# evroon/mav-detection

Measured on AMD Instinct MI355X. Metric: frame-pairs/sec at 1920x1080, higher is better.
Workload: dtype f32; 1 GPU; 1920x1080, batch 64 per GPU, Farneback + FoE + phi/threshold + box; global_batch=64, parallelism=frame-parallel x1, record_exchange=none (1 GPU), torch_in_process=False

## Files before the change

### include/mavflow.h

```cpp
#ifndef MAVFLOW_H
#define MAVFLOW_H

#include <stddef.h>
#include <stdint.h>

#ifdef __cplusplus
extern "C" {
#endif

#define MAV_OK 0
#define MAV_ERR_ARG (-1)
#define MAV_ERR_HIP (-2)
#define MAV_ERR_OOM (-3)
#define MAV_ERR_STATE (-4)

#define MAV_DEPTH_8U 0
#define MAV_DEPTH_16U 2
#define MAV_DEPTH_32F 5

typedef struct mav_ctx mav_ctx;

#define MAV_OPTFLOW_USE_INITIAL_FLOW 4
#define MAV_OPTFLOW_FARNEBACK_GAUSSIAN 256
typedef struct {
// ... 219 lines not shown
                            float* corners, int* count);
int mav_good_features_score_dev(mav_ctx*, const uint8_t* gray_dev, const uint8_t* mask_dev, const mav_gftt_params*, const mav_corner_score*,
                                float* corners_dev, int32_t* count_dev);
int mav_gftt_last_pick(mav_ctx*, uint32_t* stats);
#define MAV_LK_HIST_BINS 104
int mav_lk_last_iterations(mav_ctx*, uint32_t* hist);
int mav_lk_level_dims(const mav_ctx*, int level, int* w, int* h);

int mav_timer_start(mav_ctx*);
int mav_timer_stop(mav_ctx*, float* ms);
int mav_profile_enable(mav_ctx*, int on);
int mav_profile_get(mav_ctx*, int* n, const char** names, double* total_ms, long* launches);
int mav_profile_busy(mav_ctx*, const char* names, double* busy_ms);
int mav_profile_intervals(mav_ctx*, int* n, int* kernel_class, int* stream, float* t0_ms, float* t1_ms);

int mav_membw_probe(mav_ctx*, size_t bytes_per_buffer, int reps, double* gbs);

int mav_runtime_info(char* buf, size_t cap);
int mav_comm_unique_id(void* id128 );
int mav_comm_init(mav_ctx*, const void* id128, int rank, int nranks, void** comm_out);
int mav_comm_count(void* comm, int* nranks);
int mav_comm_destroy(void* comm);
int mav_allgather_results(mav_ctx*, void* comm, const void* local_dev, size_t bytes_per_rank, void* all_dev);

int mav_stage_blur_resize(mav_ctx*, const uint8_t* img, int k, float* out);
int mav_stage_blur_resize_two_pass(mav_ctx*, const uint8_t* img, int k, float* out);
int mav_stage_blur_resize_ex(mav_ctx*, const void* img, int depth, int k, int two_pass, float* out);
int mav_stage_polyexp(mav_ctx*, const float* I, int k, float* R);
int mav_stage_update_matrices(mav_ctx*, const float* R0, const float* R1, const float* flow, int k, float* M);
int mav_stage_update_matrices_from(mav_ctx*, const float* R0, const float* R1, const float* flow_coarse, int k, float* M);
int mav_stage_initial_flow(mav_ctx*, const float* flow0, int k, float* out);
int mav_stage_blur_iter(mav_ctx*, const float* R0, const float* R1, const float* M, int k, int update, float* flow,
                        float* M_out);

int mav_stage_phi_mask(mav_ctx*, const float* flow, const double* foe, const double* omega, const double* dt, const uint8_t* sky,
                       int batch, const mav_thr_params*, double* phi, uint8_t* mask_fixed, uint8_t* mask_dyn, int32_t* box);

int mav_stage_coefficients(mav_ctx*, int k, float* g, float* xg, float* xxg, float* ig, float* blur_taps);

int mav_stage_pyramid_level(mav_ctx*, const uint8_t* img, double scale, int level, uint8_t* out);

int mav_stage_lk_pyramid(mav_ctx*, const uint8_t* img, int level, uint8_t* out);
int mav_stage_lk_scharr(mav_ctx*, const uint8_t* img, int level, int16_t* out);
int mav_stage_min_eigen(mav_ctx*, const uint8_t* img, int block_size, float* out);
int mav_stage_corner_response(mav_ctx*, const uint8_t* img, int block_size, const mav_corner_score*, float* out);
int mav_stage_corner_pick(mav_ctx*, const uint64_t* keys, int n, const mav_gftt_params*, float* corners, int* count);

#ifdef __cplusplus
}
#endif
#endif
```

### mav-detection_amd/csrc/kernels_flow.hip

```cpp
#include "mavflow_internal.h"

#include <algorithm>
#include <type_traits>

static __device__ __forceinline__ int clampi(int v, int lo, int hi) { return v < lo ? lo : (v > hi ? hi : v); }

struct TileMap { int tiles_x, tiles_y, per_img, n_tiles, strip_w, xcd, ty0; };
static __device__ __forceinline__ bool tile_of_block(const TileMap& tm, int* s, int* tx, int* ty)
{
    const int per = ((int)gridDim.x + 7) >> 3;
    const int tile = tm.xcd ? (int)(blockIdx.x & 7) * per + (int)(blockIdx.x >> 3) : (int)blockIdx.x;
    if (tile >= tm.n_tiles) return false;
    const int img = tile / tm.per_img;
    int tr = tile - img * tm.per_img;
    const int strip_tiles = tm.strip_w * tm.tiles_y;
    const int st = tr / strip_tiles;
    tr -= st * strip_tiles;
    const int x_base = st * tm.strip_w;
    const int sw = min(tm.strip_w, tm.tiles_x - x_base);
    const int row = tr / sw;
    *s = img; *ty = row + tm.ty0; *tx = x_base + tr - row * sw;
    return true;
}
static TileMap make_tile_map(int w, int h, int G, int tile_w, int tile_h, int ty0 = 0, int ty1 = -1, int strip = 0)
// ... 1438 lines not shown
{
    const bool wt = a.write_through && a.do_update;
    const auto k = wt ? k_blur_iter_fast<Win, 6, AL, true> : k_blur_iter_fast<Win, 6, AL, false>;
    hipLaunchKernelGGL(k, dim3(tile_grid(tm)), dim3(256), 0, st, a.M_in, a.M_out, a.M_stride, a.R0, a.R1, a.R_stride, a.w, a.h, tm, win,
                       a.do_update, a.store_flow, a.flow, a.f_stride);
}

template <typename Win>
static void launch_sweep(hipStream_t st, const SweepArgs& a, const Win& win)
{
    const int m = a.winsize / 2;
    if (m == 6 && blur_iter_vec_ok(a)) {
        const TileMap tm = make_tile_map(a.w, a.h, a.G, FT_X, FT_Y, a.ty0, a.ty1, a.strip);
        if (tm.n_tiles == 0) return;
        return launch_sweep_fast<Win, true>(st, tm, a, win);
    }
    if (m == 6 && a.f_stride % 2 == 0 && ((uintptr_t)a.flow & 7) == 0)
        return launch_sweep_fast<Win, false>(st, make_tile_map(a.w, a.h, a.G, FT_X, FT_Y, 0, -1, a.strip), a, win);
    int ext, pitch, plane;
    iter_geometry(m, &ext, &pitch, &plane);
    const size_t lds = sizeof(float) * 5 * (size_t)plane;
    const dim3 grid((a.w + MAV_TILE - 1) / MAV_TILE, (a.h + MAV_TILE - 1) / MAV_TILE, a.G);
    const auto k = m == 6 ? k_blur_iter_generic<Win, 6> : k_blur_iter_generic<Win, 0>;
    hipLaunchKernelGGL(k, grid, dim3(256), lds, st, a.M_in, a.M_out, a.M_stride, a.R0, a.R1, a.R_stride, a.w, a.h, m, pitch, plane, win,
                       a.do_update, a.flow, a.f_stride);
}

void launch_blur_iter(hipStream_t st, const SweepArgs& a)
{
    if (a.gauss) launch_sweep(st, a, GaussWindow{*a.gauss});
    else launch_sweep(st, a, BoxWindow{(float)(1.0 / ((double)a.winsize * a.winsize))});
}

const char* blur_iter_prepare(int winsize)
{
    const size_t lds = blur_iter_lds_bytes(winsize);
    if (lds <= (size_t)64 * 1024) return nullptr;
    hipError_t e = hipFuncSetAttribute((const void*)k_blur_iter_generic<BoxWindow, 0>, hipFuncAttributeMaxDynamicSharedMemorySize, (int)lds);
    if (e == hipSuccess) e = hipFuncSetAttribute((const void*)k_blur_iter_generic<GaussWindow, 0>, hipFuncAttributeMaxDynamicSharedMemorySize, (int)lds);
    return e == hipSuccess ? nullptr : hipGetErrorString(e);
}

__global__ __launch_bounds__(256) void k_probe_r3w1(const float4* __restrict__ a, const float4* __restrict__ b, const float4* __restrict__ c,
                                                    float4* __restrict__ d, size_t n)
{
    for (size_t i = (size_t)blockIdx.x * 256 + threadIdx.x; i < n; i += (size_t)gridDim.x * 256) {
        const float4 x = a[i], y = b[i], z = c[i];
        d[i] = make_float4(x.x + y.x + z.x, x.y + y.y + z.y, x.z + y.z + z.z, x.w + y.w + z.w);
    }
}
void launch_probe_r3w1(hipStream_t st, const float* a, const float* b, const float* c, float* d, size_t n_float4)
{
    hipLaunchKernelGGL(k_probe_r3w1, dim3(256 * 8), dim3(256), 0, st, (const float4*)a, (const float4*)b, (const float4*)c, (float4*)d, n_float4);
}
```

### mav-detection_amd/csrc/mavflow.cpp

```cpp
#include <assert.h>
#include <dlfcn.h>
#include <math.h>
#include <float.h>
#include <stdarg.h>
#include <stdio.h>
#include <stdlib.h>
#include <string.h>

#include <algorithm>
#include <atomic>
#include <condition_variable>
#include <deque>
#include <map>
#include <mutex>
#include <string>
#include <thread>
#include <vector>

#include "mavflow_internal.h"

static thread_local std::string g_err;
static int fail(int code, const char* fmt, ...)
{
    char buf[512];
// ... 305 lines not shown
    mav_fb_params fb;
    hipStream_t stream = nullptr;
    hipStream_t copy_stream = nullptr;
    hipEvent_t copy_done = nullptr, compute_mark = nullptr;
    hipEvent_t gather_done = nullptr;
    struct Stager* stager = nullptr;
    struct Worker* worker = nullptr;
    int upload_threads = 4;
    bool inline_uploads = false;
    int stream_priority = 0;
    const float* last_flow = nullptr;
    const uint8_t *last_mf = nullptr, *last_md = nullptr;
    int last_mask_batch = 0;
    std::vector<Layer> layers;
    PolyCoef pc;
    size_t n0 = 0, n1 = 0;
    struct WorkSet {
        float *Htmp = nullptr;
        float *I = nullptr, *R = nullptr, *Ma = nullptr, *Mb = nullptr, *fc[2] = {nullptr, nullptr};
        float *Ic = nullptr, *Rc = nullptr;
    } ws;
    std::vector<size_t> c_off, c_stride;
    size_t c_total = 0;
    struct DeepSet { float *I = nullptr, *R = nullptr, *Ma = nullptr, *Mb = nullptr, *f[2] = {nullptr, nullptr}; } deep;
    int kd = 0, deep_cap = 0;
    int deep_frac = 6;
    bool deep_batch = true;
    int band_skew = -1;
    int band_phase = 0;
    bool coarse_bands = false;
    int small_g = 0;
    bool small_batch = true;
    int sweep_wt = -1;
    int small_batch_mb = 200;
    int window = MAV_WINDOW_BOX;
    GaussTaps gauss;
    int bands = 1;
    int pairs_in_flight = 2, pif_band_mb = 96;
    bool bands_set = false;
    int bands_auto = 1;
    bool group_fine_set = false;
    hipStream_t pair_stream = nullptr;
    hipEvent_t pif_fork = nullptr, pif_join = nullptr;
    bool share_frames = true;
    int coarse_cache_mb = 220;
    bool share_m = true;
    int coarse_half = 0;
    int strip = 0;
    bool phi_screen = true;
    int phi_yloop = 0;
    size_t htmp_stride = 0;
    DevMem mem;
    bool ws_ready = false;
    float* flow_ws = nullptr;
    float* init_snap = nullptr;
    int init_cap = 0;
    size_t init_stride = 0;
    FoeScratch foe_sc{nullptr, nullptr, nullptr};
    int foe_sc_n = 0;
    double* foe_dev = nullptr;
    int32_t* box_acc = nullptr;
    unsigned long long* u64_scratch = nullptr;
    int* i32_scratch = nullptr;
    DerotParams* derot_dev = nullptr;
    unsigned long long* render_max = nullptr;
    DerotParams* render_derot = nullptr;
// ... 320 lines not shown
}
struct Option {
    const char* name;
    long lo, hi;
    int mav_ctx::*i;
    bool mav_ctx::*b;
    bool in_schedule;
    int (*set)(mav_ctx*, long);
};
static const long kAny = 1L << 40;
static const Option kOptions[] = {
    {"group", 1, 1 << 20, &mav_ctx::group, nullptr, true, set_group},
    {"group_fine", 0, 1 << 20, &mav_ctx::group_fine, nullptr, true, set_group_fine},
    {"bands", 0, 8, &mav_ctx::bands, nullptr, true, set_bands},
    {"pairs_in_flight", 1, 2, &mav_ctx::pairs_in_flight, nullptr, true, nullptr},
    {"band_mb", 8, 1 << 20, &mav_ctx::pif_band_mb, nullptr, true, nullptr},
    {"coarse_cache_mb", 0, 1 << 20, &mav_ctx::coarse_cache_mb, nullptr, true, nullptr},
    {"coarse_half", 0, 1 << 20, &mav_ctx::coarse_half, nullptr, true, nullptr},
    {"share_m", 0, 1, nullptr, &mav_ctx::share_m, true, nullptr},
    {"share_frames", 0, 1, nullptr, &mav_ctx::share_frames, true, nullptr},
    {"strip", 0, 1 << 20, &mav_ctx::strip, nullptr, true, nullptr},
    {"phi_screen", 0, 1, nullptr, &mav_ctx::phi_screen, true, nullptr},
    {"phi_yloop", 0, 1 << 20, &mav_ctx::phi_yloop, nullptr, true, nullptr},
    {"small_batch", 0, 1, nullptr, &mav_ctx::small_batch, true, nullptr},
    {"sweep_write_through", -1, 1, &mav_ctx::sweep_wt, nullptr, true, nullptr},
    {"deep_batch", 0, 1, nullptr, &mav_ctx::deep_batch, true, nullptr},
    {"coarse_bands", 0, 1, nullptr, &mav_ctx::coarse_bands, true, nullptr},
    {"band_phase", 0, 64, &mav_ctx::band_phase, nullptr, true, nullptr},
    {"band_skew", -1, 64, &mav_ctx::band_skew, nullptr, true, nullptr},
    {"deep_frac", 1, 1 << 20, &mav_ctx::deep_frac, nullptr, true, set_deep_frac},
    {"upload_threads", 1, 64, &mav_ctx::upload_threads, nullptr, false, set_upload_threads},
    {"inline_uploads", -kAny, kAny, nullptr, &mav_ctx::inline_uploads, false, set_inline_uploads},
    {"stream_priority", -kAny, kAny, &mav_ctx::stream_priority, nullptr, false, set_stream_priority},
};
static const Option* find_option(const char* name)
{
    for (const Option& o : kOptions) if (!strcmp(o.name, name)) return &o;
    return nullptr;
}
static long option_value(const mav_ctx* c, const Option& o) { return o.i ? (long)(c->*o.i) : (long)(c->*o.b); }
extern "C" int mav_get_option(mav_ctx* c, const char* name, long* value)
{
    if (!c || !name || !value) return fail(MAV_ERR_ARG, "mav_get_option: NULL argument");
    const Option* o = find_option(name);
    if (!o) return fail(MAV_ERR_ARG, "unknown option '%s'", name);
    *value = option_value(c, *o);
    return MAV_OK;
}
extern "C" int mav_set_option(mav_ctx* c, const char* name, long value)
{
    if (!c || !name) return fail(MAV_ERR_ARG, "mav_set_option: NULL argument");
    const Option* o = find_option(name);
    if (!o) return fail(MAV_ERR_ARG, "unknown option '%s'", name);
    if (value < o->lo || value > o->hi) return fail(MAV_ERR_ARG, "option '%s' must be in [%ld, %ld], got %ld", name, o->lo, o->hi, value);
    if (o->set) return o->set(c, value);
    if (o->i) c->*o->i = (int)value; else c->*o->b = value != 0;
    return MAV_OK;
}

static const GaussTaps* window_taps(const mav_ctx* c) { return c->window == MAV_WINDOW_GAUSSIAN ? &c->gauss : nullptr; }
extern "C" int mav_set_window(mav_ctx* c, int window)
{
    if (!c) return fail(MAV_ERR_ARG, "mav_set_window: NULL context");
    if (window != MAV_WINDOW_BOX && window != MAV_WINDOW_GAUSSIAN)
        return fail(MAV_ERR_ARG, "mav_set_window: window must be MAV_WINDOW_BOX (0) or MAV_WINDOW_GAUSSIAN (1), got %d", window);
    HIPCHK(hipSetDevice(c->device));
// ... 431 lines not shown
    const Layer& l = c->layers[k];
    const int T = blur_iter_tile_rows(l.h), I = c->fb.iterations;
    auto wt = [&](int streams) { return c->sweep_wt < 0 ? streams == 2 : c->sweep_wt != 0; };
    int sub = g;
    if (k == 0 && c->group_fine > 0 && c->group_fine < g) sub = c->group_fine;
    if (k > 0 && c->coarse_cache_mb > 0) {
        const size_t ws = (size_t)l.w * l.h * 80, cap = (size_t)c->coarse_cache_mb << 20;
        const int fit = (int)(cap / (ws ? ws : 1));
        if (fit < sub) sub = fit > 1 ? fit : 1;
    }
    bool m_per_sub = sub < g;
    const size_t ws_pair = (size_t)l.w * l.h * 80, band_bytes = (size_t)c->pif_band_mb << 20;
    const bool big_coarse = k > 0 && c->coarse_bands && bands_ok && ws_pair > band_bytes && T / (I + 2) >= 2;
    if (big_coarse) { sub = 1; m_per_sub = true; }
    if (k > 0 && !big_coarse && c->pairs_in_flight == 2 && g >= 2) {
        int half = sub / 2 > 0 ? sub / 2 : 1;
        if (c->coarse_half > 0) half = c->coarse_half;
        if (2 * half > g) half = (g + 1) / 2;
        return {"two sub-groups in flight", half, 2, 1, false, M_SUB, SLOT_ALTERNATE, wt(2)};
    }
    if ((k == 0 || big_coarse) && c->pairs_in_flight == 2 && m_per_sub && sub == 1 && g >= 2) {
        int J = (c->bands_set && k == 0) ? c->bands : (int)((ws_pair + band_bytes - 1) / band_bytes);
        const int Jmax = T / (I + 2);
        if (J > Jmax) J = Jmax;
        if (J < 1) J = 1;
        if (J == 1 || bands_ok)
            return {"two pairs in flight, band-major", 1, 2, J, J > 1 && c->band_phase && J >= c->band_phase, J > 1 ? M_BAND : M_SUB,
                    SLOT_ALTERNATE, wt(2)};
    }
    const int J = (k == 0 && (m_per_sub || g == 1) && sub == 1 && T >= (I + 2) * c->bands && bands_ok) ? c->bands : 1;
    return {"one stream", sub, 1, J, false, m_per_sub ? M_SUB : M_GROUP, (m_per_sub && c->share_m) ? SLOT_FIRST : SLOT_OWN, wt(1)};
}

struct BandRun { float *Ma, *Mb; int kid , J, phase; };
static void sweeps_band_major(mav_ctx* c, hipStream_t st, SweepArgs a, const BandRun& run, const FlowSource* upd)
{
    const int I = c->fb.iterations, T = blur_iter_tile_rows(a.h), phase = run.phase;
    int J = run.J;
    const int NBands = phase ? J + 1 : J;
    auto bound = [&](int j) -> int {
        if (j <= 0) return 0;
        if (j >= NBands) return T;
        if (phase) return (int)((long long)T * (2 * j - 1) / (2 * J));
        int b = (int)((long long)T * j / J) + (c->band_skew < 0 ? (I - 1) / 2 : c->band_skew);
        const int lo = j, hi = T - (NBands - j);
        return b < lo ? lo : (b > hi ? hi : b);
    };
    J = NBands;
    for (int j = 0; j < J; j++) {
        const int a0 = bound(j), a1 = bound(j + 1);
        if (a1 <= a0) continue;
        if (upd) {
            ProfScope ps(c, K_UPDATE, st);
            launch_initial_m(st, {a, run.Ma, a.M_stride, a0 == 0 ? 0 : a0 * 16 - 8, j == J - 1 ? a.h : a1 * 16 + 8}, *upd);
        }
        for (int it = 0; it < I; it++) {
            const int update = it < I - 1;
            int ty0 = a0 - it, ty1 = j == J - 1 ? T : a1 - it;
            if (ty0 < 0) ty0 = 0;
            if (ty1 <= ty0) continue;
            ProfScope ps(c, run.kid, st);
            a.M_in = (it & 1) ? run.Mb : run.Ma; a.M_out = (it & 1) ? run.Ma : run.Mb;
            a.do_update = update; a.store_flow = !update; a.ty0 = ty0; a.ty1 = ty1;
            launch_blur_iter(st, a);
        }
    }
}

struct LayerIO { int k, g; const float *r0, *r1; size_t rs; float* flow; size_t fstride, ms; };
struct MBuffers { float *a, *b; };
static int layer_sweeps(mav_ctx* c, hipStream_t st, const LayerIO& io, const FlowSource& src, const MBuffers& m)
{
    const int k = io.k, g = io.g;
    const Layer& l = c->layers[k];
    const size_t ms = io.ms, rs = io.rs;
    const PairOperands group{io.r0, io.r1, rs, g, l.w, l.h};
    SweepArgs sa{group, m.a, m.b, ms, c->fb.winsize, io.flow, io.fstride, 1, 0};
    sa.strip = c->strip; sa.gauss = window_taps(c);
    const SweepPlan p = plan_sweeps(c, k, g, blur_iter_bands_ok(sa));
    sa.write_through = p.write_through;
    if (p.streams == 2) {
        CHK(ensure_pair_stream(c));
        HIPCHK(hipEventRecord(c->pif_fork, st));
        HIPCHK(hipStreamWaitEvent(c->pair_stream, c->pif_fork, 0));
    }
    if (p.m_build == M_GROUP) {
        ProfScope ps(c, K_UPDATE, st);
        launch_initial_m(st, {group, m.a, ms}, src);
    }
    for (int s0 = 0, i = 0; s0 < g; s0 += p.per_launch, i++) {
        const int gs = g - s0 < p.per_launch ? g - s0 : p.per_launch;
        const bool second = p.streams == 2 && (i & 1);
        const hipStream_t ss = second ? c->pair_stream : st;
        const size_t m_off = p.m_slot == SLOT_OWN ? (size_t)s0 * ms : p.m_slot == SLOT_FIRST ? 0 : (size_t)(i & 1) * p.per_launch * ms;
        sa.R0 = io.r0 + (size_t)s0 * rs; sa.R1 = io.r1 + (size_t)s0 * rs; sa.G = gs;
        sa.flow = io.flow + (size_t)s0 * io.fstride;
        const FlowSource bu = src.from_pair(s0);
        if (p.m_build == M_SUB) {
            ProfScope ps(c, K_UPDATE, ss);
            launch_initial_m(ss, {sa, m.a + m_off, ms}, bu);
        }
        sweeps_band_major(c, ss, sa, {m.a + m_off, m.b + m_off, k == 0 ? K_ITER : K_ITER_COARSE, p.J, p.shift_second && second},
                          p.m_build == M_BAND ? &bu : nullptr);
    }
    if (p.streams == 2) {
        prof_close_stream(c, c->pair_stream); prof_close_stream(c, st);
        HIPCHK(hipEventRecord(c->pif_join, c->pair_stream));
        HIPCHK(hipStreamWaitEvent(st, c->pif_join, 0));
    }
    return MAV_OK;
}

template <typename T>
static void layer_expansions(mav_ctx* c, hipStream_t st, int k, const T* prev, const T* next, int g, bool seq, float* I, float* R,
                             const float** r0, const float** r1)
{
    mav_ctx::WorkSet& w = c->ws;
    const size_t n0 = c->n0;
    const Layer& l = c->layers[k];
    const LayerTarget target{I, n0, blur_of(c, l), l.w, l.h};
    const BlurScratch scratch{w.Htmp, c->htmp_stride};
    auto frames = [&](const T* a, const T* b, int split, int G) { return FrameRun<T>{a, b, split, n0, G, c->W, c->H}; };
    if (seq) {
        { ProfScope ps(c, K_BLUR_RESIZE, st);
          launch_blur_resize(st, frames(prev, nullptr, 0, g + 1), target, scratch); }
        { ProfScope ps(c, K_POLYEXP, st);
          launch_polyexp(st, I, n0, g + 1, l.w, l.h, c->pc, R, 5 * n0); }
        *r0 = R; *r1 = R + 5 * n0;
        return;
    }
    float* R1 = R + 5 * n0 * (size_t)g;
    *r0 = R; *r1 = R1;
    const bool no_tmp = !blur_resize_needs_tmp(frames(prev, next, g, 2 * g), target);
    const bool merge_frames = (no_tmp || 2 * g <= g + 1) && (size_t)2 * g * l.w * l.h * sizeof(float) <= ((size_t)48 << 20);
    if (merge_frames) {
// ... 1530 lines not shown
    const Layer* l;
    CHK(h.fresh_layer(k, &l));
    if (!flow0 || !out) return fail(MAV_ERR_ARG, "mav_stage_initial_flow: NULL argument");
    const size_t n = (size_t)l->w * l->h;
    double scale = 1;
    for (int i = 0; i < k; i++) scale *= c->fb.pyr_scale;
    const float* di = h.in(flow0, 2 * c->n0 * sizeof(float));
    float* dout = h.out(out, 2 * n * sizeof(float));
    CHK(h.staged());
    launch_area_resize_flow(c->stream, di, 2 * c->n0, c->W, c->H, dout, 2 * n, l->w, l->h, 1, scale);
    CHK(check_launch("area_resize_flow"));
    return h.finish();
}
extern "C" int mav_stage_blur_iter(mav_ctx* c, const float* R0, const float* R1, const float* M, int k, int update, float* flow, float* M_out)
{
    HostCall h(c, "mav_stage_blur_iter");
    const Layer* l;
    CHK(h.fresh_layer(k, &l));
    if (!R0 || !R1 || !M || !flow || (update && !M_out)) return fail(MAV_ERR_ARG, "mav_stage_blur_iter: NULL argument");
    const size_t n = (size_t)l->w * l->h;
    const float* d0 = h.in(R0, 5 * n * sizeof(float));
    const float* d1 = h.in(R1, 5 * n * sizeof(float));
    const float* dm = h.in(M, 5 * n * sizeof(float));
    float* dmo = h.scratch<float>(5 * n * sizeof(float));
    float* df = h.out(flow, 2 * n * sizeof(float));
    h.fetch(update ? M_out : nullptr, dmo, 5 * n * sizeof(float));
    CHK(h.staged());
    SweepArgs a{{d0, d1, 5 * n, 1, l->w, l->h}, dm, dmo, 5 * n, c->fb.winsize, df, 2 * n, update, 1};
    a.strip = c->strip; a.gauss = window_taps(c);
    launch_blur_iter(c->stream, a);
    CHK(check_launch("blur_iter"));
    return h.finish();
}

typedef int (*nccl_get_uid_t)(void*);
struct uid128 { char b[128]; };
typedef int (*nccl_init_rank2_t)(void**, int, uid128, int);
typedef int (*nccl_destroy_t)(void*);
typedef int (*nccl_allgather_t)(const void*, void*, size_t, int, void*, hipStream_t);
typedef const char* (*nccl_errstr_t)(int);
static void* g_rccl = nullptr;
static int rccl_sym(const char* name, void** fn)
{
    if (!g_rccl) {
        g_rccl = dlopen("librccl.so.1", RTLD_NOW | RTLD_GLOBAL);
        if (!g_rccl) g_rccl = dlopen("librccl.so", RTLD_NOW | RTLD_GLOBAL);
        if (!g_rccl) return fail(MAV_ERR_STATE, "cannot load RCCL: %s", dlerror());
    }
    *fn = dlsym(g_rccl, name);
    if (!*fn) return fail(MAV_ERR_STATE, "RCCL symbol %s missing", name);
    return MAV_OK;
}
typedef int (*nccl_get_version_t)(int*);
extern "C" int mav_runtime_info(char* buf, size_t cap)
{
    if (!buf || cap < 16) return fail(MAV_ERR_ARG, "mav_runtime_info: NULL argument");
    int rt = 0, drv = 0, nccl = 0;
    if (hipRuntimeGetVersion(&rt) != hipSuccess) rt = -1;
    if (hipDriverGetVersion(&drv) != hipSuccess) drv = -1;
    void* fn = nullptr;
    if (g_rccl && (fn = dlsym(g_rccl, "ncclGetVersion"))) ((nccl_get_version_t)fn)(&nccl);
    snprintf(buf, cap, "{\"built_with_hip\": \"%d.%d.%d\", \"hip_runtime\": %d, \"hip_runtime_major\": %d, \"hip_driver\": %d, \"rccl\": %d}",
             HIP_VERSION_MAJOR, HIP_VERSION_MINOR, HIP_VERSION_PATCH, rt, rt > 0 ? rt / 10000000 : -1, drv, nccl);
    return MAV_OK;
}
extern "C" int mav_comm_unique_id(void* id128)
// ... 479 lines not shown
```

### mav-detection_amd/csrc/mavflow_internal.h

```cpp
#pragma once
#include <hip/hip_runtime.h>
#include <stdint.h>

#include "../../include/mavflow.h"

#define MAV_MAX_POLY_N 16
#define MAV_TILE 32

struct PolyCoef {
    int n;
    float g[MAV_MAX_POLY_N + 1], xg[MAV_MAX_POLY_N + 1], xxg[MAV_MAX_POLY_N + 1];
    float ig11, ig03, ig33, ig55;
};

struct BlurParams {
    int ksize;
    int fixed3;
    const float* g;
    double scale_x;
    double scale_y;
    const int* xs; const float* xf;
    const int* ys; const float* yf;
};

// ... 38 lines not shown
    Kind kind = ZERO;
    const float* flow = nullptr;
    size_t stride = 0;
    int pw = 0, ph = 0;
    float mul = 0.f;
    static FlowSource coarser(const float* flow, size_t stride, int pw, int ph, float mul)
    {
        return flow ? FlowSource{COARSER, flow, stride, pw, ph, mul} : FlowSource{};
    }
    static FlowSource field(const float* flow, size_t stride) { return FlowSource{FIELD, flow, stride}; }
    FlowSource from_pair(int s0) const { FlowSource u = *this; if (u.flow) u.flow += (size_t)s0 * stride; return u; }
};
struct InitialMArgs : PairOperands {
    float* M;
    size_t M_stride;
    int y_begin = 0, y_end = -1;
};
void launch_initial_m(hipStream_t st, const InitialMArgs& a, const FlowSource& src);
#define MAV_MAX_WIN_HALF 32
struct GaussTaps { float k[MAV_MAX_WIN_HALF + 1]; };
void gauss_taps(int winsize, GaussTaps* out);
struct SweepArgs : PairOperands {
    const float* M_in;
    float* M_out;
    size_t M_stride;
    int winsize;
    float* flow;
    size_t f_stride;
    int do_update, store_flow;
    int ty0 = 0, ty1 = -1;
    int strip = 0;
    bool write_through = false;
    const GaussTaps* gauss = nullptr;
};
void launch_blur_iter(hipStream_t st, const SweepArgs& a);
int blur_iter_tile_rows(int h);
bool blur_iter_bands_ok(const SweepArgs& a);
size_t blur_iter_lds_bytes(int winsize);
const char* blur_iter_prepare(int winsize);

void launch_probe_r3w1(hipStream_t st, const float* a, const float* b, const float* c, float* d, size_t n_float4);

struct FoeScratch {
    double* cand;
    int* count;
    unsigned long long* best_key;
    unsigned* done;
};
void launch_foe_f32(hipStream_t st, const float* flow, const DerotParams* derot , const uint32_t* samples,
                    int B, int W, int H, int N, double mag2_thr, float mag2_thr_f32 , double dist2_thr,
                    FoeScratch s, double* foe, int32_t* box_acc ,
                    unsigned long long* max_phi_bits );
void launch_foe_f64(hipStream_t st, const double* flow, const uint32_t* samples, int B, int W, int H, int N, double mag2_thr,
                    double dist2_thr, FoeScratch s, double* foe, int32_t* box_acc, unsigned long long* max_phi_bits);
void launch_box_init(hipStream_t st, int32_t* box_acc, unsigned long long* max_phi_bits, unsigned* done , int B);
struct PhiLaunch {
    unsigned* done = nullptr;
    mav_result* results = nullptr;
    int32_t* box_out = nullptr;
    bool screen = true;
    int yloop = 0;
};
void launch_phi_mask_f32(hipStream_t st, const float* flow, const DerotParams* derot, const double* foe, const uint8_t* sky,
                         int B, int W, int H, mav_thr_params thr, double* phi, uint8_t* mask_fixed, uint8_t* mask_dyn,
                         int32_t* box_acc, unsigned long long* max_phi_bits, const PhiLaunch& pl);
void launch_phi_mask_f64(hipStream_t st, const double* flow, const double* foe, const uint8_t* sky, int B, int W, int H,
                         mav_thr_params thr, double* phi, uint8_t* mask_fixed, uint8_t* mask_dyn, int32_t* box_acc,
                         unsigned long long* max_phi_bits, const PhiLaunch& pl);
// ... 91 lines not shown
```

### mav-detection_amd/mavflow/_lib.py

```python
from __future__ import annotations

import ctypes as C
import os

import numpy as np

HERE = os.path.dirname(os.path.abspath(__file__))
SO_PATH = os.path.join(HERE, "libmavflow.so")

MAV_OK, MAV_ERR_ARG, MAV_ERR_HIP, MAV_ERR_OOM, MAV_ERR_STATE = 0, -1, -2, -3, -4


class MavflowError(RuntimeError):
    """HIP / device failure inside libmavflow (the counterpart of cv2.error at the flow-operator seam)."""


class FbParams(C.Structure):
    _fields_ = [("pyr_scale", C.c_double), ("levels", C.c_int), ("winsize", C.c_int), ("iterations", C.c_int),
                ("poly_n", C.c_int), ("poly_sigma", C.c_double), ("flags", C.c_int)]


class FoeParams(C.Structure):
    _fields_ = [("n_pairs", C.c_int), ("mag_threshold", C.c_double), ("ransac_threshold", C.c_double)]

# ... 21 lines not shown

class Result(C.Structure):
    _fields_ = [("box", C.c_int32 * 4), ("foe", C.c_double * 2)]


RESULT_DTYPE = np.dtype([("box", np.int32, (4,)), ("foe", np.float64, (2,))])
assert RESULT_DTYPE.itemsize == C.sizeof(Result) == 32

EXPORTS = [
    "mav_fb_defaults", "mav_foe_defaults", "mav_thr_defaults", "mav_create", "mav_destroy", "mav_last_error",
    "mav_device_count", "mav_set_option", "mav_num_layers", "mav_layer_dims", "mav_farneback", "mav_derotate",
    "mav_foe_dense", "mav_ransac", "mav_bgr2gray", "mav_phi_mask", "mav_bbox", "mav_window_max", "mav_tpr_fpr_counts", "mav_process_batch",
    "mav_farneback_dev", "mav_process_batch_dev", "mav_sync", "mav_stream", "mav_dev_alloc", "mav_dev_free",
    "mav_memcpy_h2d", "mav_memcpy_d2h", "mav_host_alloc", "mav_host_free", "mav_upload_async", "mav_upload_fence", "mav_timer_start", "mav_timer_stop", "mav_profile_enable", "mav_profile_get", "mav_profile_busy",
    "mav_comm_unique_id", "mav_comm_init", "mav_comm_destroy", "mav_allgather_results", "mav_stage_blur_resize",
    "mav_stage_polyexp", "mav_stage_update_matrices", "mav_stage_blur_iter",
    "mav_analyze_pyramid", "mav_pyramid_levels", "mav_pyramid_dims", "mav_optimize_window", "mav_stage_pyramid_level",
    "mav_detect", "mav_detect_dev", "mav_last_flow_dev", "mav_foe_dense_f32", "mav_phi_mask_f32", "mav_stage_coefficients",
    "mav_stage_phi_mask", "mav_last_masks_tpr_fpr", "mav_get_option", "mav_schedule_info", "mav_stage_blur_resize_two_pass",
    "mav_membw_probe", "mav_runtime_info", "mav_upload_async_unordered", "mav_mem_info", "mav_profile_intervals",
    "mav_upload_gather", "mav_download_async", "mav_marker_create", "mav_marker_record", "mav_marker_wait", "mav_marker_destroy",
    "mav_tpr_fpr_counts_dev", "mav_bgr2gray_dev", "mav_png_unfilter", "mav_comm_count",
    "mav_marker_query", "mav_frame_step_dev", "mav_frame_step_post", "mav_frame_step_wait", "mav_worker_drain", "mav_worker_wait_enqueued",
    "mav_farneback_init", "mav_farneback_init_dev", "mav_stage_update_matrices_from", "mav_stage_initial_flow",
    "mav_farneback_ex", "mav_farneback_ex_dev", "mav_stage_blur_resize_ex", "mav_schedule_info_ex",
    "mav_render", "mav_render_dev", "mav_last_render", "mav_flow_to_color", "mav_colormap_jet",
    "mav_overlay", "mav_overlay_dev", "mav_last_overlay",
    "mav_png_bound", "mav_png_encode", "mav_png_encode_dev", "mav_last_render_png", "mav_last_overlay_png",
    "mav_gftt_defaults", "mav_lk_defaults", "mav_good_features", "mav_good_features_dev", "mav_lk_track", "mav_lk_track_dev",
    "mav_lk_last_iterations", "mav_lk_level_dims", "mav_stage_lk_pyramid", "mav_stage_lk_scharr", "mav_stage_min_eigen",
    "mav_good_features_ex", "mav_good_features_ex_dev", "mav_lk_track_ex_dev", "mav_gftt_last_pick", "mav_stage_corner_pick",
    "mav_set_window", "mav_get_window",
    "mav_lk_track_err", "mav_lk_track_err_dev", "mav_corner_score_defaults", "mav_good_features_score", "mav_good_features_score_dev",
    "mav_stage_corner_response",
]

DEPTH_8U, DEPTH_16U, DEPTH_32F = 0, 2, 5
DEPTHS = {np.dtype(np.uint8): DEPTH_8U, np.dtype(np.uint16): DEPTH_16U, np.dtype(np.float32): DEPTH_32F}

OPTFLOW_USE_INITIAL_FLOW = 4
OPTFLOW_LK_GET_MIN_EIGENVALS = 8
OPTFLOW_FARNEBACK_GAUSSIAN = 256
WINDOW_BOX, WINDOW_GAUSSIAN = 0, 1
WINDOWS = {"box": WINDOW_BOX, "gaussian": WINDOW_GAUSSIAN}

GATHER_ORDERED, GATHER_SOURCES_HELD = 1, 2
STEP_MAX_GATHER = 4


class Gather(C.Structure):
    _fields_ = [("src_host", C.POINTER(C.c_void_p)), ("count", C.c_int), ("bytes_each", C.c_size_t), ("dst_dev", C.c_void_p)]


class FrameStep(C.Structure):
    _fields_ = [("n", C.c_int),
                ("wait_before", C.POINTER(C.c_void_p)), ("n_wait_before", C.c_int),
                ("par_host", C.c_void_p), ("par_dev", C.c_void_p), ("par_bytes", C.c_size_t),
                ("gather", Gather * STEP_MAX_GATHER), ("n_gather", C.c_int),
                ("bgr_dev", C.c_void_p), ("n_bgr", C.c_int), ("gray_dev", C.c_void_p),
                ("compute_flow", C.c_int), ("prev_dev", C.c_void_p), ("next_dev", C.c_void_p), ("flow_dev", C.c_void_p),
                ("record_after_flow", C.POINTER(C.c_void_p)), ("n_record_after_flow", C.c_int),
                ("detect", C.c_int),
                ("off_samples", C.c_size_t), ("off_omega", C.c_size_t), ("off_dt", C.c_size_t), ("off_frame0", C.c_size_t),
                ("has_omega", C.c_int), ("has_frame0", C.c_int),
                ("sky_dev", C.c_void_p), ("gt_dev", C.c_void_p), ("gt_images", C.c_int),
                ("foe", FoeParams), ("thr", ThrParams),
                ("mask_fixed_dev", C.c_void_p), ("mask_dyn_dev", C.c_void_p), ("out_dev", C.c_void_p),
# ... 76 lines not shown
    lib.mav_upload_fence.argtypes = [vp]
    lib.mav_upload_gather.argtypes = [vp, vp, C.POINTER(vp), C.c_int, C.c_size_t, C.c_int]
    lib.mav_download_async.argtypes = [vp, vp, vp, C.c_size_t]
    lib.mav_marker_create.argtypes = [vp, C.POINTER(vp)]
    lib.mav_marker_record.argtypes = [vp, vp]
    lib.mav_marker_wait.argtypes = [vp, vp]
    lib.mav_marker_destroy.argtypes = [vp, vp]
    lib.mav_marker_query.argtypes = [vp, vp, C.POINTER(C.c_int)]
    lib.mav_frame_step_dev.argtypes = [vp, C.POINTER(FrameStep)]
    lib.mav_frame_step_post.argtypes = [vp, C.POINTER(FrameStep), C.POINTER(C.c_uint64)]
    lib.mav_frame_step_wait.argtypes = [vp, C.c_uint64, vp]
    lib.mav_worker_drain.argtypes = [vp]
    lib.mav_worker_wait_enqueued.argtypes = [vp, C.c_uint64]
    lib.mav_tpr_fpr_counts_dev.argtypes = [vp, vp, C.c_int, vp, vp, C.c_int, C.c_int, vp, vp]
    lib.mav_bgr2gray_dev.argtypes = [vp, vp, C.c_int, vp]
    lib.mav_png_unfilter.argtypes = [vp, C.c_int, C.c_size_t, C.c_int, vp]
    lib.mav_timer_start.argtypes = [vp]
    lib.mav_timer_stop.argtypes = [vp, C.POINTER(C.c_float)]
    lib.mav_profile_enable.argtypes = [vp, C.c_int]
    lib.mav_profile_get.argtypes = [vp, C.POINTER(C.c_int), C.POINTER(C.c_char_p), C.POINTER(C.c_double), C.POINTER(C.c_long)]
    lib.mav_profile_busy.argtypes = [vp, C.c_char_p, C.POINTER(C.c_double)]
    lib.mav_profile_intervals.argtypes = [vp, C.POINTER(C.c_int), vp, vp, vp, vp]
    lib.mav_comm_unique_id.argtypes = [vp]
    lib.mav_comm_init.argtypes = [vp, vp, C.c_int, C.c_int, C.POINTER(vp)]
    lib.mav_comm_destroy.argtypes = [vp]
    lib.mav_comm_count.argtypes = [vp, C.POINTER(C.c_int)]
    lib.mav_allgather_results.argtypes = [vp, vp, vp, C.c_size_t, vp]
    lib.mav_stage_blur_resize.argtypes = [vp, vp, C.c_int, vp]
    lib.mav_stage_blur_resize_two_pass.argtypes = [vp, vp, C.c_int, vp]
    lib.mav_stage_polyexp.argtypes = [vp, vp, C.c_int, vp]
    lib.mav_stage_update_matrices.argtypes = [vp, vp, vp, vp, C.c_int, vp]
    lib.mav_stage_blur_iter.argtypes = [vp, vp, vp, vp, C.c_int, C.c_int, vp, vp]
    lib.mav_stage_update_matrices_from.argtypes = [vp, vp, vp, vp, C.c_int, vp]
    lib.mav_stage_initial_flow.argtypes = [vp, vp, C.c_int, vp]
    lib.mav_farneback_ex.argtypes = [vp, vp, vp, C.c_int, C.c_int, vp, vp]
    lib.mav_farneback_ex_dev.argtypes = [vp, vp, vp, C.c_int, C.c_int, vp, vp]
    lib.mav_stage_blur_resize_ex.argtypes = [vp, vp, C.c_int, C.c_int, C.c_int, vp]
    lib.mav_schedule_info_ex.argtypes = [vp, C.c_int, C.c_int, C.c_char_p, C.c_size_t]
    rn = [vp, vp, vp, vp, vp, vp, vp, C.c_int, C.POINTER(ThrParams), vp, vp, vp]
    lib.mav_render.argtypes = rn
    lib.mav_render_dev.argtypes = rn
    lib.mav_last_render.argtypes = [vp, C.c_int, vp, vp, vp]
    lib.mav_flow_to_color.argtypes = [vp, vp, C.c_int, C.c_int, vp]
    lib.mav_colormap_jet.argtypes = [vp, vp, C.c_size_t, vp]
    lib.mav_overlay.argtypes = [vp, vp, vp, vp, vp, C.c_int, C.c_int, vp, vp]
    lib.mav_overlay_dev.argtypes = [vp, vp, vp, vp, vp, C.c_int, C.c_int, vp, vp]
    lib.mav_last_overlay.argtypes = [vp, vp, vp, C.c_int, C.c_int, vp, vp]
    lib.mav_png_bound.argtypes = [C.c_int, C.c_int, C.c_int]
    lib.mav_png_bound.restype = C.c_size_t
    lib.mav_png_encode.argtypes = [vp, vp, C.c_int, C.c_int, vp, C.c_size_t, vp]
    lib.mav_png_encode_dev.argtypes = [vp, vp, C.c_int, C.c_int, vp, C.c_size_t, vp]
    lib.mav_last_render_png.argtypes = [vp, C.c_int, C.c_int, C.c_int, C.c_int, vp, C.c_size_t, vp]
    lib.mav_last_overlay_png.argtypes = [vp, vp, vp, C.c_int, C.c_int, vp, C.c_size_t, vp, vp]
    lib.mav_gftt_defaults.argtypes = [C.POINTER(GfttParams)]
    lib.mav_lk_defaults.argtypes = [C.POINTER(LkParams)]
    lib.mav_good_features.argtypes = [vp, vp, C.POINTER(GfttParams), vp, C.POINTER(C.c_int)]
    lib.mav_good_features_dev.argtypes = [vp, vp, C.POINTER(GfttParams), vp, C.POINTER(C.c_int)]
    lib.mav_lk_track.argtypes = [vp, vp, vp, vp, C.c_int, C.POINTER(LkParams), vp, vp]
    lib.mav_lk_track_dev.argtypes = [vp, vp, vp, vp, C.c_int, C.POINTER(LkParams), vp, vp]
    lib.mav_lk_last_iterations.argtypes = [vp, vp]
    lib.mav_lk_level_dims.argtypes = [vp, C.c_int, C.POINTER(C.c_int), C.POINTER(C.c_int)]
    lib.mav_stage_lk_pyramid.argtypes = [vp, vp, C.c_int, vp]
    lib.mav_stage_lk_scharr.argtypes = [vp, vp, C.c_int, vp]
    lib.mav_stage_min_eigen.argtypes = [vp, vp, C.c_int, vp]
    lib.mav_good_features_ex.argtypes = [vp, vp, vp, C.POINTER(GfttParams), vp, C.POINTER(C.c_int)]
    lib.mav_good_features_ex_dev.argtypes = [vp, vp, vp, C.POINTER(GfttParams), vp, vp]
# ... 994 lines not shown
        w, h, _, _ = self.layer_dims(k)
        R0 = _arr(R0, np.float32, (5, h, w), "R0"); R1 = _arr(R1, np.float32, (5, h, w), "R1")
        flow = _arr(flow, np.float32, (h, w, 2), "flow")
        M = np.empty((5, h, w), np.float32)
        check(self.lib.mav_stage_update_matrices(self.h, _ptr(R0), _ptr(R1), _ptr(flow), k, _ptr(M)))
        return M

    def stage_update_matrices_from(self, R0, R1, flow_coarse, k):
        w, h, _, _ = self.layer_dims(k)
        R0 = _arr(R0, np.float32, (5, h, w), "R0"); R1 = _arr(R1, np.float32, (5, h, w), "R1")
        if flow_coarse is not None:
            pw, ph = (self.layer_dims(k + 1)[:2] if k + 1 < self.num_layers() else np.shape(flow_coarse)[1::-1])
            flow_coarse = _arr(flow_coarse, np.float32, (ph, pw, 2), "flow_coarse")
        M = np.empty((5, h, w), np.float32)
        check(self.lib.mav_stage_update_matrices_from(self.h, _ptr(R0), _ptr(R1), _ptr(flow_coarse), k, _ptr(M)))
        return M

    def stage_initial_flow(self, flow0, k):
        flow0 = _arr(flow0, np.float32, (self.H, self.W, 2), "flow0")
        w, h, _, _ = self.layer_dims(k)
        out = np.empty((h, w, 2), np.float32)
        check(self.lib.mav_stage_initial_flow(self.h, _ptr(flow0), k, _ptr(out)))
        return out

    def stage_blur_iter(self, R0, R1, M, k, update=True):
        w, h, _, _ = self.layer_dims(k)
        R0 = _arr(R0, np.float32, (5, h, w), "R0"); R1 = _arr(R1, np.float32, (5, h, w), "R1")
        M = _arr(M, np.float32, (5, h, w), "M")
        flow = np.empty((h, w, 2), np.float32)
        Mo = np.empty((5, h, w), np.float32)
        check(self.lib.mav_stage_blur_iter(self.h, _ptr(R0), _ptr(R1), _ptr(M), k, int(bool(update)), _ptr(flow), _ptr(Mo)))
        return flow, (Mo if update else None)


def runtime_info() -> dict:
    import json
    buf = C.create_string_buffer(512)
    check(load().mav_runtime_info(buf, len(buf)))
    return json.loads(buf.value.decode())


def device_count() -> int:
    return load().mav_device_count()
```

Baseline: 2661 frame-pairs/s.

## Carry flow instead of M matrices between Farneback sweep iterations

```diff
diff --git a/include/mavflow.h b/include/mavflow.h
--- a/include/mavflow.h
+++ b/include/mavflow.h
@@ -275,6 +275,7 @@
 int mav_stage_initial_flow(mav_ctx*, const float* flow0, int k, float* out);
 int mav_stage_blur_iter(mav_ctx*, const float* R0, const float* R1, const float* M, int k, int update, float* flow,
                         float* M_out);
+int mav_stage_sweep_flow(mav_ctx*, const float* R0, const float* R1, const float* flow_in, int k, float* flow_out);
 
 int mav_stage_phi_mask(mav_ctx*, const float* flow, const double* foe, const double* omega, const double* dt, const uint8_t* sky,
                        int batch, const mav_thr_params*, double* phi, uint8_t* mask_fixed, uint8_t* mask_dyn, int32_t* box);
diff --git a/mav-detection_amd/csrc/kernels_flow.hip b/mav-detection_amd/csrc/kernels_flow.hip
--- a/mav-detection_amd/csrc/kernels_flow.hip
+++ b/mav-detection_amd/csrc/kernels_flow.hip
@@ -1494,6 +1494,176 @@
     else launch_sweep(st, a, BoxWindow{(float)(1.0 / ((double)a.winsize * a.winsize))});
 }
 
+#ifndef FC_X
+#define FC_X 60
+#endif
+#ifndef FC_GI
+#define FC_GI 2
+#endif
+template <typename Win, int M_T, int TW, bool AL>
+__global__ __launch_bounds__(256, 4) void k_sweep_flow(const float* __restrict__ F_in, size_t fin_stride, const float* __restrict__ R0,
+                                                       const float* __restrict__ R1, size_t R_stride, int w, int h, TileMap tm, Win win,
+                                                       float* __restrict__ F_out, size_t fout_stride)
+{
+    constexpr int EXT_X = TW + 2 * M_T;
+    constexpr int EXT_Y = FT_Y + 2 * M_T;
+    constexpr int PITCH = EXT_X;
+    constexpr int PLANE = EXT_Y * PITCH + (EXT_X - (EXT_Y * PITCH) % 32 + 64) % 32;
+    constexpr int NPX = EXT_X * EXT_Y;
+    constexpr int NR = (NPX + 255) / 256;
+    constexpr int GI = FC_GI;
+    static_assert(TW % 4 == 0 && TW <= 64 && PLANE % 4 == 0, "tile width: a multiple of 4, at most one wave of columns");
+    __shared__ __attribute__((aligned(16))) float vs[5 * PLANE];
+    const int tid = threadIdx.x;
+    const int lane = tid & 63, wv = tid >> 6;
+    int s, tx, ty;
+    if (!tile_of_block(tm, &s, &tx, &ty)) return;
+    const int x0 = tx * TW, y0 = ty * FT_Y;
+    const size_t npx = (size_t)w * h;
+    const float* Fi = F_in + (size_t)s * fin_stride;
+    const float* R0p = R0 + (size_t)s * R_stride;
+    const float* R1p = R1 + (size_t)s * R_stride;
+
+    auto ext_px = [&](int r, int* lx, int* ly, int* gx, int* gy) {
+        const int p = min(tid + 256 * r, NPX - 1);
+        *ly = p / EXT_X; *lx = p - *ly * EXT_X;
+        *gx = clampi(x0 - M_T + *lx, 0, w - 1); *gy = clampi(y0 - M_T + *ly, 0, h - 1);
+    };
+    float2 fl[NR];
+#pragma unroll
+    for (int r = 0; r < NR; r++) {
+        int lx, ly, gx, gy;
+        ext_px(r, &lx, &ly, &gx, &gy);
+        fl[r] = *(const float2*)(Fi + ((size_t)gy * w + gx) * 2);
+    }
+#pragma unroll
+    for (int rb = 0; rb < NR; rb += GI) {
+        GatherPx g[GI];
+        float q[GI][5];
+#pragma unroll
+        for (int jj = 0; jj < GI; jj++) {
+            if (rb + jj >= NR) continue;
+            int lx, ly, gx, gy;
+            ext_px(rb + jj, &lx, &ly, &gx, &gy);
+            const size_t idx = (size_t)gy * w + gx;
+#pragma unroll
+            for (int c = 0; c < 5; c++) q[jj][c] = R0p[c * npx + idx];
+            gather_issue(R1p, npx, w, h, gx, gy, fl[rb + jj].x, fl[rb + jj].y, g[jj]);
+        }
+#pragma unroll
+        for (int jj = 0; jj < GI; jj++) {
+            if (rb + jj >= NR) continue;
+            int lx, ly, gx, gy;
+            ext_px(rb + jj, &lx, &ly, &gx, &gy);
+            float o[5];
+            update_finish(q[jj], g[jj], w, h, gx, gy, fl[rb + jj].x, fl[rb + jj].y, o);
+            if (tid + 256 * (rb + jj) < NPX) {
+#pragma unroll
+                for (int c = 0; c < 5; c++) vs[c * PLANE + ly * PITCH + lx] = o[c];
+            }
+        }
+    }
+    __syncthreads();
+
+    {
+        constexpr int NP = EXT_X / 2;
+        for (int t = tid; t < 5 * NP; t += 256) {
+            const int c = t / NP, pr = t - c * NP;
+            float* col = vs + c * PLANE + 2 * pr;
+            float2 v[EXT_Y];
+#pragma unroll
+            for (int i = 0; i < EXT_Y; i++) v[i] = *(const float2*)(col + i * PITCH);
+            win.template sums<M_T, FT_Y, true>(M_T, [&](int i) { return v[i]; }, [&](int y, float2 a) { *(float2*)(col + y * PITCH) = a; });
+        }
+    }
+    __syncthreads();
+
+    const int quad = (lane & 31) >> 2;
+    const int grp = (lane >> 5) * 2 + ((quad == 1 || quad == 2 || quad == 4 || quad == 7) ? 1 : 0);
+    const int qpos = (quad == 0 || quad == 1) ? 0 : ((quad == 3 || quad == 2) ? 1 : ((quad == 5 || quad == 4) ? 2 : 3));
+    const int pos = qpos * 4 + (lane & 3);
+    const int ly = wv * 4 + grp;
+    const int lx0 = pos * 4;
+    const int gx = x0 + lx0, gy = y0 + ly;
+    if (lx0 >= TW || gx >= w || gy >= h) return;
+    float S[5][4];
+#pragma unroll
+    for (int c = 0; c < 5; c++) {
+        const float4* p = (const float4*)(vs + c * PLANE + ly * PITCH + lx0);
+        constexpr int NV = (4 + 2 * M_T + 3) / 4;
+        float f[4 * NV];
+#pragma unroll
+        for (int k = 0; k < NV; k++) {
+            const float4 t4 = p[k];
+            f[4 * k] = t4.x; f[4 * k + 1] = t4.y; f[4 * k + 2] = t4.z; f[4 * k + 3] = t4.w;
+        }
+        win.template sums<M_T, 4, true>(M_T, [&](int i) { return f[i]; }, [&](int j, float a) { S[c][j] = a; });
+    }
+    float u[4], v[4];
+#pragma unroll
+    for (int j = 0; j < 4; j++) win.solve(S[0][j], S[1][j], S[2][j], S[3][j], S[4][j], &u[j], &v[j]);
+    float* fo = F_out + (size_t)s * fout_stride + ((size_t)gy * w + gx) * 2;
+    if (AL) {
+#ifdef FC_WT
+#pragma unroll
+        for (int j = 0; j < 4; j++) {
+            const unsigned long long b = (unsigned long long)__float_as_uint(u[j]) | ((unsigned long long)__float_as_uint(v[j]) << 32);
+            __hip_atomic_store((unsigned long long*)(fo + 2 * j), b, __ATOMIC_RELAXED, __HIP_MEMORY_SCOPE_AGENT);
+        }
+#else
+        *(float4*)fo = make_float4(u[0], v[0], u[1], v[1]);
+        *(float4*)(fo + 4) = make_float4(u[2], v[2], u[3], v[3]);
+#endif
+    } else {
+#pragma unroll
+        for (int j = 0; j < 4; j++)
+            if (gx + j < w) *(float2*)(fo + 2 * j) = make_float2(u[j], v[j]);
+    }
+}
+
+static bool aligned8(const void* p) { return ((uintptr_t)p & 7) == 0; }
+bool sweep_flow_ok(const SweepArgs& a)
+{
+    return a.winsize / 2 == 6 && a.flow_in && a.flow && a.fin_stride % 2 == 0 && a.f_stride % 2 == 0 && aligned8(a.flow_in) && aligned8(a.flow);
+}
+template <typename Win>
+static void launch_sweep_flow_win(hipStream_t st, const SweepArgs& a, const Win& win)
+{
+    const bool al = a.w % 4 == 0 && a.f_stride % 4 == 0 && aligned16(a.flow);
+    const TileMap tm = make_tile_map(a.w, a.h, a.G, FC_X, FT_Y, a.ty0, a.ty1, a.strip);
+    if (tm.n_tiles == 0) return;
+    const auto k = al ? k_sweep_flow<Win, 6, FC_X, true> : k_sweep_flow<Win, 6, FC_X, false>;
+    hipLaunchKernelGGL(k, dim3(tile_grid(tm)), dim3(256), 0, st, a.flow_in, a.fin_stride, a.R0, a.R1, a.R_stride, a.w, a.h, tm, win, a.flow,
+                       a.f_stride);
+}
+void launch_sweep_flow(hipStream_t st, const SweepArgs& a)
+{
+    if (a.gauss) launch_sweep_flow_win(st, a, GaussWindow{*a.gauss});
+    else launch_sweep_flow_win(st, a, BoxWindow{(float)(1.0 / ((double)a.winsize * a.winsize))});
+}
+
+template <int MODE>
+__global__ __launch_bounds__(256) void k_initial_flow(const float* __restrict__ fsrc, size_t f_stride, int pw, int ph, float mul, double scale_x,
+                                                      double scale_y, int w, int h, float* __restrict__ F, size_t F_stride, int y_begin, int y_end)
+{
+    const int x = blockIdx.x * 64 + (threadIdx.x & 63);
+    const int y = y_begin + blockIdx.y * 4 + (threadIdx.x >> 6);
+    if (x >= w || y >= y_end) return;
+    const int s = blockIdx.z;
+    float2 f = make_float2(0.f, 0.f);
+    if (MODE == 1) f = upsample_flow(fsrc + (size_t)s * f_stride, pw, ph, mul, scale_x, scale_y, x, y);
+    else if (MODE == 2) f = *(const float2*)(fsrc + (size_t)s * f_stride + ((size_t)y * w + x) * 2);
+    *(float2*)(F + (size_t)s * F_stride + ((size_t)y * w + x) * 2) = f;
+}
+void launch_initial_flow(hipStream_t st, const InitialFlowArgs& a, const FlowSource& src)
+{
+    const int y_begin = a.y_begin < 0 ? 0 : a.y_begin, y_end = (a.y_end < 0 || a.y_end > a.h) ? a.h : a.y_end;
+    if (y_end <= y_begin) return;
+    const auto k = src.kind == FlowSource::COARSER ? k_initial_flow<1> : src.kind == FlowSource::FIELD ? k_initial_flow<2> : k_initial_flow<0>;
+    hipLaunchKernelGGL(k, dim3((a.w + 63) / 64, (y_end - y_begin + 3) / 4, a.G), dim3(256), 0, st, src.flow, src.stride, src.pw, src.ph, src.mul,
+                       (double)src.pw / a.w, (double)src.ph / a.h, a.w, a.h, a.F, a.F_stride, y_begin, y_end);
+}
+
 const char* blur_iter_prepare(int winsize)
 {
     const size_t lds = blur_iter_lds_bytes(winsize);
diff --git a/mav-detection_amd/csrc/mavflow.cpp b/mav-detection_amd/csrc/mavflow.cpp
--- a/mav-detection_amd/csrc/mavflow.cpp
+++ b/mav-detection_amd/csrc/mavflow.cpp
@@ -361,6 +361,7 @@
     int small_g = 0;
     bool small_batch = true;
     int sweep_wt = -1;
+    int sweep_carry = -1;
     int small_batch_mb = 200;
     int window = MAV_WINDOW_BOX;
     GaussTaps gauss;
@@ -747,6 +748,7 @@
     {"upload_threads", 1, 64, &mav_ctx::upload_threads, nullptr, false, set_upload_threads},
     {"inline_uploads", -kAny, kAny, nullptr, &mav_ctx::inline_uploads, false, set_inline_uploads},
     {"stream_priority", -kAny, kAny, &mav_ctx::stream_priority, nullptr, false, set_stream_priority},
+    {"sweep_carry", -1, 1, &mav_ctx::sweep_carry, nullptr, false, nullptr},
 };
 static const Option* find_option(const char* name)
 {
@@ -1244,7 +1246,7 @@
     return {"one stream", sub, 1, J, false, m_per_sub ? M_SUB : M_GROUP, (m_per_sub && c->share_m) ? SLOT_FIRST : SLOT_OWN, wt(1)};
 }
 
-struct BandRun { float *Ma, *Mb; int kid , J, phase; };
+struct BandRun { float *Ma, *Mb; int kid , J, phase; bool carry; };
 static void sweeps_band_major(mav_ctx* c, hipStream_t st, SweepArgs a, const BandRun& run, const FlowSource* upd)
 {
     const int I = c->fb.iterations, T = blur_iter_tile_rows(a.h), phase = run.phase;
@@ -1264,7 +1266,9 @@
         if (a1 <= a0) continue;
         if (upd) {
             ProfScope ps(c, K_UPDATE, st);
-            launch_initial_m(st, {a, run.Ma, a.M_stride, a0 == 0 ? 0 : a0 * 16 - 8, j == J - 1 ? a.h : a1 * 16 + 8}, *upd);
+            const int y_begin = a0 == 0 ? 0 : a0 * 16 - 8, y_end = j == J - 1 ? a.h : a1 * 16 + 8;
+            if (run.carry) launch_initial_flow(st, {a.G, a.w, a.h, run.Ma, a.M_stride, y_begin, y_end}, *upd);
+            else launch_initial_m(st, {a, run.Ma, a.M_stride, y_begin, y_end}, *upd);
         }
         for (int it = 0; it < I; it++) {
             const int update = it < I - 1;
@@ -1274,6 +1278,13 @@
             ProfScope ps(c, run.kid, st);
             a.M_in = (it & 1) ? run.Mb : run.Ma; a.M_out = (it & 1) ? run.Ma : run.Mb;
             a.do_update = update; a.store_flow = !update; a.ty0 = ty0; a.ty1 = ty1;
+            if (run.carry) {
+                SweepArgs f = a;
+                f.flow_in = a.M_in; f.fin_stride = a.M_stride;
+                if (update) { f.flow = a.M_out; f.f_stride = a.M_stride; }
+                launch_sweep_flow(st, f);
+                continue;
+            }
             launch_blur_iter(st, a);
         }
     }
@@ -1281,6 +1292,13 @@
 
 struct LayerIO { int k, g; const float *r0, *r1; size_t rs; float* flow; size_t fstride, ms; };
 struct MBuffers { float *a, *b; };
+static bool sweeps_carry_flow(const mav_ctx* c, const SweepPlan& p, const SweepArgs& a)
+{
+    SweepArgs f = a;
+    f.flow_in = a.M_in; f.fin_stride = a.M_stride;
+    if (!sweep_flow_ok(f) || ((uintptr_t)a.M_out & 7) != 0) return false;
+    return c->sweep_carry < 0 ? p.streams == 2 : c->sweep_carry != 0;
+}
 static int layer_sweeps(mav_ctx* c, hipStream_t st, const LayerIO& io, const FlowSource& src, const MBuffers& m)
 {
     const int k = io.k, g = io.g;
@@ -1291,6 +1309,11 @@
     sa.strip = c->strip; sa.gauss = window_taps(c);
     const SweepPlan p = plan_sweeps(c, k, g, blur_iter_bands_ok(sa));
     sa.write_through = p.write_through;
+    const bool carry = sweeps_carry_flow(c, p, sa);
+    auto initial = [&](hipStream_t s, const SweepArgs& a, float* Ma, const FlowSource& from) {
+        if (carry) launch_initial_flow(s, {a.G, a.w, a.h, Ma, ms}, from);
+        else launch_initial_m(s, {a, Ma, ms}, from);
+    };
     if (p.streams == 2) {
         CHK(ensure_pair_stream(c));
         HIPCHK(hipEventRecord(c->pif_fork, st));
@@ -1298,7 +1321,7 @@
     }
     if (p.m_build == M_GROUP) {
         ProfScope ps(c, K_UPDATE, st);
-        launch_initial_m(st, {group, m.a, ms}, src);
+        initial(st, sa, m.a, src);
     }
     for (int s0 = 0, i = 0; s0 < g; s0 += p.per_launch, i++) {
         const int gs = g - s0 < p.per_launch ? g - s0 : p.per_launch;
@@ -1310,9 +1333,9 @@
         const FlowSource bu = src.from_pair(s0);
         if (p.m_build == M_SUB) {
             ProfScope ps(c, K_UPDATE, ss);
-            launch_initial_m(ss, {sa, m.a + m_off, ms}, bu);
+            initial(ss, sa, m.a + m_off, bu);
         }
-        sweeps_band_major(c, ss, sa, {m.a + m_off, m.b + m_off, k == 0 ? K_ITER : K_ITER_COARSE, p.J, p.shift_second && second},
+        sweeps_band_major(c, ss, sa, {m.a + m_off, m.b + m_off, k == 0 ? K_ITER : K_ITER_COARSE, p.J, p.shift_second && second, carry},
                           p.m_build == M_BAND ? &bu : nullptr);
     }
     if (p.streams == 2) {
@@ -2909,6 +2932,27 @@
     CHK(check_launch("blur_iter"));
     return h.finish();
 }
+extern "C" int mav_stage_sweep_flow(mav_ctx* c, const float* R0, const float* R1, const float* flow_in, int k, float* flow_out)
+{
+    HostCall h(c, "mav_stage_sweep_flow");
+    const Layer* l;
+    CHK(h.fresh_layer(k, &l));
+    if (!R0 || !R1 || !flow_in || !flow_out) return fail(MAV_ERR_ARG, "mav_stage_sweep_flow: NULL argument");
+    if (c->fb.winsize / 2 != 6) return fail(MAV_ERR_ARG, "mav_stage_sweep_flow: the flow-carried sweep exists for winsize 12 and 13, not %d", c->fb.winsize);
+    const size_t n = (size_t)l->w * l->h;
+    const float* d0 = h.in(R0, 5 * n * sizeof(float));
+    const float* d1 = h.in(R1, 5 * n * sizeof(float));
+    const float* dfi = h.in(flow_in, 2 * n * sizeof(float));
+    float* df = h.out(flow_out, 2 * n * sizeof(float));
+    CHK(h.staged());
+    SweepArgs a{{d0, d1, 5 * n, 1, l->w, l->h}, nullptr, nullptr, 0, c->fb.winsize, df, 2 * n, 0, 1};
+    a.strip = c->strip; a.gauss = window_taps(c);
+    a.flow_in = dfi; a.fin_stride = 2 * n;
+    if (!sweep_flow_ok(a)) return fail(MAV_ERR_STATE, "mav_stage_sweep_flow: staged flow fields are not 8-byte aligned");
+    launch_sweep_flow(c->stream, a);
+    CHK(check_launch("sweep_flow"));
+    return h.finish();
+}
 
 typedef int (*nccl_get_uid_t)(void*);
 struct uid128 { char b[128]; };
diff --git a/mav-detection_amd/csrc/mavflow_internal.h b/mav-detection_amd/csrc/mavflow_internal.h
--- a/mav-detection_amd/csrc/mavflow_internal.h
+++ b/mav-detection_amd/csrc/mavflow_internal.h
@@ -94,8 +94,14 @@
     int strip = 0;
     bool write_through = false;
     const GaussTaps* gauss = nullptr;
+    const float* flow_in = nullptr;
+    size_t fin_stride = 0;
 };
 void launch_blur_iter(hipStream_t st, const SweepArgs& a);
+void launch_sweep_flow(hipStream_t st, const SweepArgs& a);
+bool sweep_flow_ok(const SweepArgs& a);
+struct InitialFlowArgs { int G, w, h; float* F; size_t F_stride; int y_begin = 0, y_end = -1; };
+void launch_initial_flow(hipStream_t st, const InitialFlowArgs& a, const FlowSource& src);
 int blur_iter_tile_rows(int h);
 bool blur_iter_bands_ok(const SweepArgs& a);
 size_t blur_iter_lds_bytes(int winsize);
diff --git a/mav-detection_amd/mavflow/_lib.py b/mav-detection_amd/mavflow/_lib.py
--- a/mav-detection_amd/mavflow/_lib.py
+++ b/mav-detection_amd/mavflow/_lib.py
@@ -77,7 +77,7 @@
     "mav_good_features_ex", "mav_good_features_ex_dev", "mav_lk_track_ex_dev", "mav_gftt_last_pick", "mav_stage_corner_pick",
     "mav_set_window", "mav_get_window",
     "mav_lk_track_err", "mav_lk_track_err_dev", "mav_corner_score_defaults", "mav_good_features_score", "mav_good_features_score_dev",
-    "mav_stage_corner_response",
+    "mav_stage_corner_response", "mav_stage_sweep_flow",
 ]
 
 DEPTH_8U, DEPTH_16U, DEPTH_32F = 0, 2, 5
@@ -220,6 +220,7 @@
     lib.mav_stage_update_matrices.argtypes = [vp, vp, vp, vp, C.c_int, vp]
     lib.mav_stage_blur_iter.argtypes = [vp, vp, vp, vp, C.c_int, C.c_int, vp, vp]
     lib.mav_stage_update_matrices_from.argtypes = [vp, vp, vp, vp, C.c_int, vp]
+    lib.mav_stage_sweep_flow.argtypes = [vp, vp, vp, vp, C.c_int, vp]
     lib.mav_stage_initial_flow.argtypes = [vp, vp, C.c_int, vp]
     lib.mav_farneback_ex.argtypes = [vp, vp, vp, C.c_int, C.c_int, vp, vp]
     lib.mav_farneback_ex_dev.argtypes = [vp, vp, vp, C.c_int, C.c_int, vp, vp]
@@ -1280,6 +1281,14 @@
         check(self.lib.mav_stage_blur_iter(self.h, _ptr(R0), _ptr(R1), _ptr(M), k, int(bool(update)), _ptr(flow), _ptr(Mo)))
         return flow, (Mo if update else None)
 
+    def stage_sweep_flow(self, R0, R1, flow, k):
+        w, h, _, _ = self.layer_dims(k)
+        R0 = _arr(R0, np.float32, (5, h, w), "R0"); R1 = _arr(R1, np.float32, (5, h, w), "R1")
+        flow = _arr(flow, np.float32, (h, w, 2), "flow")
+        out = np.empty((h, w, 2), np.float32)
+        check(self.lib.mav_stage_sweep_flow(self.h, _ptr(R0), _ptr(R1), _ptr(flow), k, _ptr(out)))
+        return out
+
 
 def runtime_info() -> dict:
     import json
```

New measurement: 2374 frame-pairs/s. 0.892x the previous value.
